# GAIA-vision/GAIA-seg

Hardware: AMD Instinct MI355X
Metric: supernet train images/sec at 1024x512 (higher is better)
Workload: dtype fp32

## Files before the change

### gaia_seg_amd/core/bricks.py

```python
import math
import warnings

import os

import torch
import torch.nn as nn
from torch.nn.modules.batchnorm import _BatchNorm

from ..hip import ops
from ..hip import runtime as _runtime
from ..hip.runtime import round_up, tape_function
from .dynamic import DynamicMixin
from .registry import Registry, build_from_cfg

CONV_LAYERS = Registry("conv layer")
NORM_LAYERS = Registry("norm layer")
ACTIVATION_LAYERS = Registry("activation layer")
ACTIVATION_LAYERS.register_module("ReLU", module=nn.ReLU)


def _nhwc_tape_call(run, x):
    if x.dim() != 4:
        raise ValueError("expected a [N, H, W, C] tensor (got %dD input)" % x.dim())
    return tape_function(lambda tape, acts: [run(tape, acts[0])], [x.permute(0, 3, 1, 2)],
# ... 383 lines not shown


_NO_FUSED_CALLS = os.environ.get("GS_NO_FUSED_CALLS") is not None


def fused_call_ok(conv, norm):
    return (conv._parameters["bias"] is None and conv.width_state % 4 == 0 and not conv.depthwise
            and not conv.__dict__.get("_deploying", False)
            and not norm.__dict__.get("_deploying", False) and not _NO_FUSED_CALLS
            and not (norm.training and norm.sync is not None and norm._process_group() is not None))


def conv_bn_act(tape, conv, norm, x, relu=False, residual=None, out=None, tag=None, defer=False,
                owns_input_grad=False, defer_residual=False):
    c = conv.width_state
    cd = conv.__dict__
    weight = conv._parameters["weight"]
    fused = (conv._parameters["bias"] is None and c % 4 == 0 and not cd.get("_deploying", False)
             and not cd["depthwise"]
             and not norm.__dict__.get("_deploying", False) and not _NO_FUSED_CALLS)
    if fused:
        bnp = norm.bn_params(c)
        if bnp.process_group is None:
            if cd.get("_layout_ptr") != weight.data_ptr():
                conv._check_layout()
                weight = conv._parameters["weight"]
                cd["_layout_ptr"] = weight.data_ptr()
            return ops.conv_bn(tape, x, weight, c, bnp, conv.stride, conv.padding,
                               conv.dilation, relu=relu, residual=residual, out=out, tag=tag,
                               defer=defer, owns_input_grad=owns_input_grad,
                               defer_residual=defer_residual)
    y = conv.forward_act(tape, x, tag=tag)
    return norm.forward_act(tape, y, relu=relu, residual=residual, out=out)


class DynamicConvModule(nn.Module, DynamicMixin):
    search_space = {"width"}

    def __init__(self, in_channels, out_channels, kernel_size, stride=1, padding=0, dilation=1,
                 groups=1, bias="auto", conv_cfg=None, norm_cfg=None, act_cfg=dict(type="ReLU"),
                 inplace=True, order=("conv", "norm", "act")):
        super().__init__()
        if tuple(order) != ("conv", "norm", "act"):
            raise NotImplementedError("only the conv-norm-act order is used by the heads")
        self.with_norm = norm_cfg is not None
        self.with_activation = act_cfg is not None
        if self.with_activation and act_cfg.get("type") != "ReLU":
            raise NotImplementedError("only ReLU activations are fused")
        if bias == "auto":
            bias = not self.with_norm
        self.with_bias = bias
        if self.with_norm and self.with_bias:
            warnings.warn("ConvModule has norm and bias at the same time")
        self.conv = build_conv_layer(conv_cfg, in_channels, out_channels, kernel_size,
                                     stride=stride, padding=padding, dilation=dilation,
                                     groups=groups, bias=bias)
        self.in_channels, self.out_channels = in_channels, out_channels
        self.inplace = inplace
        if self.with_norm:
            self.norm_name, norm = build_norm_layer(norm_cfg, out_channels)
            self.add_module(self.norm_name, norm)
        else:
            self.norm_name = None
        if self.with_activation:
            self.activate = nn.ReLU(inplace=inplace)
        self.init_weights()
# ... 190 lines not shown
```

### gaia_seg_amd/csrc/fused_layers.hip

```cpp
#include <vector>
#include "common.h"
#include "fused_internal.h"

using namespace gs;

static inline size_t align256(size_t v) { return (v + 255) & ~(size_t)255; }

extern "C" size_t gs_conv_bn_workspace_bytes(const gs_conv_desc* d) {
  if (!d) return 0;
  const size_t a = gs_conv2d_workspace_bytes(d);
  const int64_t rows = (int64_t)d->N * d->Ho * d->Wo;
  const size_t b = gs_bn_stats_workspace_bytes(rows, d->Co);
  const size_t fused = align256(a) + bn_fused_reduce_bytes(rows, d->Co);
  const size_t tiles = align256(a) + (size_t)3 * d->Co * ((rows + 63) / 64) * sizeof(float);
  size_t m = a > b ? a : b;
  if (fused > m) m = fused;
  if (tiles > m) m = tiles;
  const size_t bnb = dgrad_bnbwd_part_bytes(d);
  if (bnb > m) m = bnb;
  return m;
}

extern "C" int gs_conv_bn_forward(const gs_conv_desc* d, const float* x, const float* w,
                                  const gs_bn_args* bn, const float* residual, int32_t ld_res,
// ... 58 lines not shown
  if (input_bn && input_bn->reserved != 0) return GS_E_BADARG;
  const int64_t rows = (int64_t)d->N * d->Ho * d->Wo;
  const int32_t C = d->Co;
  int rc = GS_OK;
  if (!sums_ready) {
    rc = gs_bn_bwd_reduce(dz, ld_dz, y, d->ldy, z, ldz, rows, C, coeffs, mask_mode,
                          write_g ? dz : nullptr, ld_dz, bsums, workspace, workspace_bytes, stream);
    if (rc != GS_OK) return rc;
  }
  rc = gs_bn_bwd_apply(dz, ld_dz, y, d->ldy, z, ldz, rows, C, coeffs, bsums, (double)rows,
                       (write_g || sums_ready) ? 0 : mask_mode, bn->use_batch_stats, dy, d->ldy,
                       dgamma, dbeta, stream);
  if (rc != GS_OK) return rc;
  if (dw) {
    if (side_stream) {
      rc = gs_stream_fork(stream, side_stream);
      if (rc != GS_OK) return rc;
      rc = gs_conv2d_wgrad(d, x, dy, dw, side_workspace, side_workspace_bytes, side_stream);
    } else {
      rc = gs_conv2d_wgrad(d, x, dy, dw, workspace, workspace_bytes, stream);
    }
    if (rc != GS_OK) return rc;
  }
  if (input_bn && input_bn->fused) *input_bn->fused = 0;
  if (dx) {
    int fused = 0;
    rc = conv2d_dgrad_impl(d, dy, w, dx, accumulate_dx, workspace, workspace_bytes, stream, input_bn,
                           &fused);
    if (input_bn && input_bn->fused) *input_bn->fused = fused;
  }
  return rc;
}

namespace gs {
struct K3Prof {
  bool on = false;
  std::vector<hipEvent_t> pool;
  size_t used = 0;
  double flops = 0.0;
};
static K3Prof g_k3;
bool k3_prof_on() { return g_k3.on; }
static hipEvent_t k3_event() {
  if (g_k3.used == g_k3.pool.size()) {
    hipEvent_t e;
    if (hipEventCreate(&e) != hipSuccess) return nullptr;
    g_k3.pool.push_back(e);
  }
  return g_k3.pool[g_k3.used++];
}
struct K3Pending {
  hipEvent_t e0 = nullptr, e1 = nullptr;
  bool open = false, start_set = false, stop_set = false;
};
static thread_local K3Pending t_k3;
void k3_prof_begin(hipStream_t st) {
  (void)st;
  t_k3 = K3Pending{};
  t_k3.e0 = k3_event();
  t_k3.e1 = k3_event();
  t_k3.open = t_k3.e0 && t_k3.e1;
}
bool k3_launch_events(hipStream_t st, bool single_kernel, hipEvent_t* e0, hipEvent_t* e1) {
  if (!t_k3.open || t_k3.start_set) return false;
  static const bool markers = getenv("GS_K3_TIMER_MARKERS") != nullptr;
  t_k3.start_set = true;
// ... 42 lines not shown
```

### gaia_seg_amd/csrc/norm.hip

```cpp
#include <algorithm>
#include "common.h"
#include "fused_internal.h"

namespace gs {

struct ColMap {
  int cq;
  int rr;
  int rpi;
  bool active;
};

__device__ __forceinline__ ColMap col_map(int C4) {
  ColMap m;
  const int t = threadIdx.x;
  if (C4 <= 256) {
    m.rpi = 256 / C4;
    m.rr = t / C4;
    m.cq = t - m.rr * C4;
    m.active = m.rr < m.rpi;
  } else {
    m.rpi = 1;
    m.rr = 0;
    m.cq = blockIdx.y * 256 + t;
// ... 278 lines not shown
}

template <int MASK, bool BATCH>
__global__ __launch_bounds__(256) void bn_bwd_apply_kernel(
    const float* __restrict__ dy, int ld_dy, const float* __restrict__ x, int ldx,
    const float* __restrict__ act, int ld_act, long rows, int C, const float* __restrict__ coeffs,
    const float* __restrict__ sums, float inv_count, float* __restrict__ dx, int ld_dx,
    float* dgamma, float* dbeta) {
  const int C4 = C >> 2;
  const ColMap m = col_map(C4);
  if (!m.active) return;
  const f32x4 scale = *reinterpret_cast<const f32x4*>(coeffs + m.cq * 4);
  const f32x4 beta = *reinterpret_cast<const f32x4*>(coeffs + C + m.cq * 4);
  const f32x4 mean = *reinterpret_cast<const f32x4*>(coeffs + 2 * C + m.cq * 4);
  const f32x4 invstd = *reinterpret_cast<const f32x4*>(coeffs + 3 * C + m.cq * 4);
  const f32x4 sg = *reinterpret_cast<const f32x4*>(sums + m.cq * 4);
  const f32x4 sgx = *reinterpret_cast<const f32x4*>(sums + C + m.cq * 4);
  if (blockIdx.x == 0 && m.rr == 0) {
    if (dgamma) *reinterpret_cast<f32x4*>(dgamma + m.cq * 4) = sgx;
    if (dbeta) *reinterpret_cast<f32x4*>(dbeta + m.cq * 4) = sg;
  }
  const f32x4 c1 = sg * inv_count, c2 = sgx * inv_count;
  const long step = (long)gridDim.x * m.rpi;
  for (long r = (long)blockIdx.x * m.rpi + m.rr; r < rows; r += step) {
    const f32x4 xv = *reinterpret_cast<const f32x4*>(x + r * ldx + m.cq * 4);
    f32x4 g = *reinterpret_cast<const f32x4*>(dy + r * ld_dy + m.cq * 4);
    f32x4 av{0.f, 0.f, 0.f, 0.f};
    if (MASK == 2) av = *reinterpret_cast<const f32x4*>(act + r * ld_act + m.cq * 4);
    g = masked_grad<MASK>(g, xv, av, mean, scale, beta);
    f32x4 o;
    if (BATCH) o = scale * (g - c1 - ((xv - mean) * invstd) * c2);
    else o = scale * g;
    *reinterpret_cast<f32x4*>(dx + r * ld_dx + m.cq * 4) = o;
  }
}

__global__ __launch_bounds__(256) void colsum_partial_kernel(const float* __restrict__ x, long rows,
                                                             int C, int ldx, long rows_per_block,
                                                             float* __restrict__ part) {
  __shared__ f32x4 sh[512];
  const int C4 = C >> 2;
  const ColMap m = col_map(C4);
  f32x4 s1{0.f, 0.f, 0.f, 0.f}, s2{0.f, 0.f, 0.f, 0.f};
  if (m.active) {
    const long r0 = (long)blockIdx.x * rows_per_block;
    const long r1 = min(r0 + rows_per_block, rows);
    for (long r = r0 + m.rr; r < r1; r += m.rpi)
      s1 += *reinterpret_cast<const f32x4*>(x + r * ldx + m.cq * 4);
  }
  block_reduce_rows(s1, s2, m, C4, sh);
  if (m.active && m.rr == 0)
    reinterpret_cast<f32x4*>(part)[(long)m.cq * gridDim.x + blockIdx.x] = s1;
}


__device__ __forceinline__ void block_sum_d4(double (&a)[4], double* sh ) {
  const int lane = threadIdx.x & 63, wave = threadIdx.x >> 6;
#pragma unroll
  for (int off = 32; off > 0; off >>= 1)
#pragma unroll
    for (int e = 0; e < 4; ++e) a[e] += __shfl_xor(a[e], off, 64);
  __syncthreads();
  if (lane == 0)
#pragma unroll
    for (int e = 0; e < 4; ++e) sh[wave * 4 + e] = a[e];
  __syncthreads();
// ... 506 lines not shown
  hipLaunchKernelGGL(colsum_partial_kernel, dim3(g.gx, g.gy), dim3(256), 0, st, src, (long)rows, C,
                     ld, g.rows_per_block, part);
  launch_sum_partials(part, g.gx, C, out, nullptr, 0, st);
  return launch_status();
}

extern "C" int gs_bn_sync_local(const float* sums, double count, int32_t C, double* local,
                                void* stream) {
  if (!sums || !local) return GS_E_NULL;
  if (C <= 0 || count <= 0.0) return GS_E_BADARG;
  hipLaunchKernelGGL(bn_sync_local_kernel, dim3((C + 255) / 256), dim3(256), 0, as_stream(stream),
                     sums, count, C, local);
  return launch_status();
}

extern "C" int gs_bn_sync_merge(const double* gathered, int32_t world, int32_t C, float* merged,
                                void* stream) {
  if (!gathered || !merged) return GS_E_NULL;
  if (C <= 0 || world <= 0) return GS_E_BADARG;
  hipLaunchKernelGGL(bn_sync_merge_kernel, dim3((C + 255) / 256), dim3(256), 0, as_stream(stream),
                     gathered, world, C, merged);
  return launch_status();
}

extern "C" int gs_bn_calib_fold(const GsBnCalibLayer* layers, int32_t n_layers, float* bank,
                                int64_t bank_floats, int32_t op, float scale, void* stream) {
  if (!layers || !bank) return GS_E_NULL;
  if (n_layers <= 0 || bank_floats <= 0 || op < GS_BN_CALIB_SAVE || op > GS_BN_CALIB_WRITE)
    return GS_E_BADARG;
  hipLaunchKernelGGL(bn_calib_fold_kernel, dim3(n_layers), dim3(256), 0, as_stream(stream), layers,
                     bank, (long)bank_floats, (int)op, scale);
  return launch_status();
}
```

### gaia_seg_amd/hip/lib.py

```python
import ctypes
import os
import subprocess
from ctypes import (POINTER, Structure, c_char_p, c_double, c_float, c_int32, c_int64, c_size_t,
                    c_void_p)

_HERE = os.path.dirname(os.path.abspath(__file__))
PKG_ROOT = os.path.dirname(_HERE)
REPO_ROOT = os.path.dirname(PKG_ROOT)
LIB_PATH = os.path.join(PKG_ROOT, "lib", "libgaiaseg_hip.so")
CSRC_DIR = os.path.join(PKG_ROOT, "csrc")
ABI_VERSION = 21


class HipLibraryError(RuntimeError):
    pass


class ConvDesc(Structure):
    _fields_ = [("N", c_int32), ("H", c_int32), ("W", c_int32), ("Ci", c_int32), ("Co", c_int32),
                ("Ci_max", c_int32), ("Co_ld", c_int32), ("KH", c_int32), ("KW", c_int32),
                ("stride", c_int32), ("pad", c_int32), ("dil", c_int32), ("Ho", c_int32),
                ("Wo", c_int32), ("x_sn", c_int64), ("x_sh", c_int64), ("x_sw", c_int64),
                ("x_sc", c_int64), ("ldy", c_int32), ("ld_add", c_int32),
                ("role", c_int32), ("reserved", c_int32), ("in_affine", c_void_p)]
# ... 299 lines not shown
    "gs_sgd_set_hyper": (_i32, [_P, _f32, _f32, _f32, _f32, _P]),
    "gs_sgd_set_group_hyper": (_i32, [_P, _f32, _f32, _i32, SgdGroups, _P]),
    "gs_sgd_step_groups": (_i32, [_P, _P, _P, _P, _i32, _P, _i32, _P]),
    "gs_adamw_set_group_hyper": (_i32, [_P, _f64, _f64, _f64, _f64, _i32, AdamwGroups, _P]),
    "gs_adamw_step_groups": (_i32, [_P, _P, _P, _P, _P, _i32, _P, _i32, _P, _i32, _P]),
    "gs_grad_accumulate": (_i32, [_P, _P, _i64, _P]),
    "gs_debug_force_plan": (_i32, [_i32, _i32, _i32]),
    "gs_debug_query_plan": (_i32, [_i32, _i32, _i32, _i32, POINTER(_i32), POINTER(_i32), POINTER(_i32),
                                   POINTER(_i32)]),
    "gs_debug_last_conv_launch": (_i32, [POINTER(DebugLaunch)]),
    "gs_debug_conv_launch_counts": (_i32, [POINTER(_i64), _i32]),
    "gs_debug_k3_flops": (_i32, [POINTER(_f64), _i32]),
    "gs_debug_set_x3_fwd": (_i32, [_i32]),
    "gs_debug_set_splitk_inkernel": (_i32, [_i32]),
    "gs_debug_splitk_combined": (_i64, [_i32]),
    "gs_debug_set_col_finalize": (_i32, [_i32]),
    "gs_debug_col_finalized": (_i64, [_i32]),
    "gs_debug_num_cu": (_i32, []),
    "gs_debug_set_stream_mode": (_i32, [_i32]),
    "gs_debug_conv_launch_flops": (_i32, [POINTER(_f64), _i32]),
    "gs_debug_query_conv_launch": (_i32, [_CD, _i32, POINTER(DebugLaunch)]),
    "gs_debug_f16_launches": (_i32, [POINTER(_i64), POINTER(_f64), _i32]),
    "gs_set_forward_precision": (_i32, [_i32]),
    "gs_get_forward_precision": (_i32, []),
    "gs_set_train_precision": (_i32, [_i32]),
    "gs_get_train_precision": (_i32, []),
    "gs_debug_f16_launches_by_op": (_i32, [POINTER(_i64), POINTER(_f64), _i32]),
    "gs_stream_fork": (_i32, [_P, _P]),
    "gs_conv_bn_workspace_bytes": (_sz, [_CD]),
    "gs_conv_bn_forward": (_i32, [_CD, _P, _P, _BN, _P, _i32, _P, _P, _P, _i32, _P, _sz, _P]),
    "gs_conv_bn_backward": (_i32, [_CD, _P, _P, _P, _P, _i32, _P, _BN, _P, _i32, _i32, _i32, _P, _P,
                                   _P, _P, _P, _P, _i32, _P, _sz, _P, _sz, _P, _P, POINTER(BnBwdFuse),
                                   _i32]),
    "gs_k3_timer_enable": (_i32, [_i32]),
    "gs_k3_timer_read": (_i32, [POINTER(_i64), POINTER(_f64), POINTER(_f64)]),
}

_lib = None


def build(verbose=False, jobs=None):
    jobs = jobs or min(8, os.cpu_count() or 1)
    cmd = ["make", "-C", CSRC_DIR, "-j%d" % jobs]
    res = subprocess.run(cmd, stdout=subprocess.PIPE, stderr=subprocess.STDOUT, text=True)
    if verbose or res.returncode != 0:
        print(res.stdout)
    if res.returncode != 0:
        raise HipLibraryError("building libgaiaseg_hip.so failed (exit %d)" % res.returncode)
    global _lib
    _lib = None
    return LIB_PATH


def load():
    global _lib, LIB_PATH
    if _lib is not None:
        return _lib
    if os.environ.get("GS_HIP_LIB"):
        LIB_PATH = os.environ["GS_HIP_LIB"]
    if not os.path.exists(LIB_PATH):
        raise HipLibraryError(
            "%s not found: the HIP extension is required (no CPU fallback). Build it with "
            "`python -c 'import __graft_entry__ as g; g.build()'` or `make -C gaia_seg_amd/csrc`."
            % LIB_PATH)
    try:
        lib = ctypes.CDLL(LIB_PATH)
# ... 48 lines not shown
```

### gaia_seg_amd/hip/ops.py

```python
import ctypes

import torch

import os

from . import lib as _lib
from .runtime import WORKSPACE, Act, _Workspace, current_stream_ptr, round_up

_ws = WORKSPACE

class _DeviceStreams:
    __slots__ = ("side", "side_dirty", "branch", "origin", "branch_dirty")

    def __init__(self):
        self.side = None
        self.side_dirty = False
        self.branch = {}
        self.origin = {}
        self.branch_dirty = set()


_streams = {}


# ... 1231 lines not shown
        if residual is not None and residual.requires_grad:
            _pass_residual_grad(L, residual, dz, rows, C, s)

    tape.record(backward)
    return out


def maxpool(tape, x, k=3, s=2, p=1):
    L = _L()
    dev = x.t.device
    ho, wo = (x.H + 2 * p - k) // s + 1, (x.W + 2 * p - k) // s + 1
    out = Act.empty(x.N, ho, wo, x.C, dev)
    idx = torch.empty((x.N, ho, wo, x.C), dtype=torch.uint8, device=dev)
    _lib.check(L.gs_maxpool_forward(x.ptr, x.N, x.H, x.W, x.C, x.ld, k, s, p, ho, wo, out.ptr,
                                    out.ld, idx.data_ptr(), current_stream_ptr()),
               "gs_maxpool_forward")
    if POOL_TRACE is not None:
        POOL_TRACE.append(idx)

    def backward():
        dy = out.g
        if dy is None or not x.requires_grad:
            return
        acc = _input_grad(x)
        _lib.check(L.gs_maxpool_backward(dy.data_ptr(), dy.stride(2), idx.data_ptr(), x.N, x.H, x.W,
                                         x.C, k, s, p, ho, wo, x.g.data_ptr(), x.g.stride(2),
                                         acc, current_stream_ptr()),
                   "gs_maxpool_backward")

    tape.record(backward)
    return out


def avgpool_ceil(tape, x, s):
    L = _L()
    x = materialize(tape, x)
    dev = x.t.device
    ho, wo = (x.H + s - 1) // s, (x.W + s - 1) // s
    out = Act.empty(x.N, ho, wo, x.C, dev)
    _lib.check(L.gs_avgpool_ceil_forward(x.ptr, x.N, x.H, x.W, x.C, x.ld, s, out.ptr, out.ld,
                                         current_stream_ptr()), "gs_avgpool_ceil_forward")

    def backward():
        dy = out.g
        if dy is None or not x.requires_grad:
            return
        acc = _input_grad(x)
        _lib.check(L.gs_avgpool_ceil_backward(dy.data_ptr(), dy.stride(2), x.N, x.H, x.W, x.C, s,
                                              x.g.data_ptr(), x.g.stride(2), acc,
                                              current_stream_ptr()), "gs_avgpool_ceil_backward")

    tape.record(backward)
    return out


def copy_into(tape, x, dst):
    L = _L()
    _lib.check(L.gs_copy2d(x.ptr, x.ld, dst.ptr, dst.ld, x.rows, x.C, 1.0, 0, current_stream_ptr()),
               "gs_copy2d")

    def backward():
        dg = dst.g
        if dg is None or not x.requires_grad:
            return
        acc = _input_grad(x)
        _lib.check(L.gs_copy2d(dg.data_ptr(), dg.stride(2), x.g.data_ptr(), x.g.stride(2), x.rows,
# ... 143 lines not shown
```

### gaia_seg_amd/models/backbones/dynamic_resnet.py

```python
from collections.abc import Sequence

import torch.nn as nn
from torch.nn.modules.batchnorm import _BatchNorm

from ...core.bricks import (DynamicBatchNorm2d, DynamicBottleneck, DynamicConv2d,
                            build_conv_layer, build_norm_layer, constant_init, conv_bn_act, kaiming_init)
from ...core.dynamic import DynamicMixin, freeze, unzip_meta
from ...hip import ops
from ...hip.runtime import tape_function
from ..builder import BACKBONES
from ..utils import DynamicResLayer


@BACKBONES.register_module()
class DynamicResNet(nn.Module, DynamicMixin):
    search_space = {"stem", "body"}

    def init_state(self, stem=None, body=None, **kwargs):
        if stem is not None:
            self.stem_state = stem
        if body is not None:
            self.body_state = body
        for k, v in kwargs.items():
            setattr(self, "%s_state" % k, v)

    def __init__(self, in_channels, stem_width, body_width, body_depth, num_stages=4,
                 strides=(1, 2, 2, 2), dilations=(1, 1, 1, 1), out_indices=(0, 1, 2, 3),
                 style="pytorch", deep_stem=False, avg_down=False, frozen_stages=-1,
                 frozen_layers=None, conv_cfg=None, norm_cfg=dict(type="DynSyncBN"),
                 act_cfg=dict(type="ReLU"), norm_eval=False, dcn=None,
                 stage_with_dcn=(False, False, False, False), plugins=None, with_cp=False,
                 zero_init_residual=True, contract_dilation=False):
        super().__init__()
        if not 1 <= num_stages <= 4:
            raise AssertionError("num_stages must be in 1..4")
        if not (len(strides) == len(dilations) == num_stages) or max(out_indices) >= num_stages:
            raise AssertionError("strides / dilations / out_indices do not match num_stages")
        if dcn is not None or plugins is not None:
            raise NotImplementedError("dcn / plugins are not used by the in-tree seg configs")
# ... 81 lines not shown
            raise TypeError("pretrained must be a str or None")
        last_norms = {id(m.norm3) for m in self.modules()
                      if isinstance(m, DynamicBottleneck)} if self.zero_init_residual else set()
        for m in self.modules():
            if isinstance(m, DynamicConv2d):
                kaiming_init(m)
            elif isinstance(m, (_BatchNorm, nn.GroupNorm)):
                constant_init(m, 0 if id(m) in last_norms else 1)

    def train(self, mode=True):
        super().train(mode)
        self._freeze_stages()
        if mode and self.norm_eval:
            for m in self.modules():
                if isinstance(m, _BatchNorm):
                    m.eval()
        return self

    def _stem_convs(self):
        return [self.stem[0], self.stem[3], self.stem[6]] if self.deep_stem else [self.conv1]

    def manipulate_stem(self, arch_meta):
        self.stem_state = arch_meta
        metas = unzip_meta(arch_meta) if self.deep_stem else [arch_meta]
        for conv, meta in zip(self._stem_convs(), metas):
            conv.manipulate_arch(meta)

    def manipulate_body(self, arch_meta):
        self.body_state = arch_meta
        for name, meta in zip(self.res_layers, unzip_meta(arch_meta)):
            getattr(self, name).manipulate_arch(meta)

    def forward_act(self, tape, x):
        if self.deep_stem:
            mods = list(self.stem)
            for i in range(0, len(mods), 3):
                x = conv_bn_act(tape, mods[i], mods[i + 1], x, relu=True)
        else:
            x = conv_bn_act(tape, self.conv1, self.norm1, x, relu=True)
        mp = self.maxpool
        x = ops.maxpool(tape, x, mp.kernel_size, mp.stride, mp.padding)
        outs = []
        for i, layer_name in enumerate(self.res_layers):
            x = getattr(self, layer_name).forward_act(tape, x)
            if i == 0:
                ops.side_checkpoint(tape)
            if i in self.out_indices:
                outs.append(x)
        return outs

    def late_gradient_parameters(self):
        mods = [self.stem] if self.deep_stem else [self.conv1, self.norm1]
        mods.append(getattr(self, self.res_layers[0]))
        return [p for m in mods for p in m.parameters()]

    def forward(self, x):
        needs = any(p.requires_grad for p in self.parameters())
        return tuple(tape_function(lambda tape, acts: self.forward_act(tape, acts[0]), [x], needs))

    def active_modules(self):
        mods = [self.stem] if self.deep_stem else [self.conv1, self.norm1]
        for layer_name in self.res_layers:
            mods.extend(getattr(self, layer_name).active_blocks())
        return mods
```

### include/gaiaseg_hip.h

```cpp
#ifndef GAIASEG_HIP_H
#define GAIASEG_HIP_H

#include <stddef.h>
#include <stdint.h>

#ifdef __cplusplus
extern "C" {
#endif

#define GS_OK 0
#define GS_E_BADARG (-1)
#define GS_E_ALIGN (-2)
#define GS_E_WORKSPACE (-3)
#define GS_E_NULL (-4)

int gs_abi_version(void);
const char* gs_error_string(int code);
const char* gs_target_arch(void);

typedef struct gs_conv_desc {
  int32_t N, H, W;
  int32_t Ci, Co;
  int32_t Ci_max, Co_ld;
  int32_t KH, KW;
// ... 102 lines not shown
size_t gs_bn_stats_workspace_bytes(int64_t rows, int32_t C);
int gs_bn_stats(const float* x, int64_t rows, int32_t C, int32_t ldx, float* sums,
                void* workspace, size_t workspace_bytes, void* stream);
int gs_bn_finalize(const float* sums, double count, int32_t C, const float* gamma,
                   const float* beta, float eps, float momentum, float* running_mean,
                   float* running_var, float* coeffs, void* stream);
int gs_bn_sync_local(const float* sums, double count, int32_t C, double* local, void* stream);
int gs_bn_sync_merge(const double* gathered, int32_t world, int32_t C, float* merged, void* stream);
int gs_bn_stats_finalize(const float* x, int64_t rows, int32_t C, int32_t ldx, const float* gamma,
                         const float* beta, float eps, float momentum, float* running_mean,
                         float* running_var, float* coeffs, void* workspace,
                         size_t workspace_bytes, void* stream);
int gs_bn_eval_coeffs(const float* running_mean, const float* running_var, int32_t C,
                      const float* gamma, const float* beta, float eps, float* coeffs,
                      void* stream);
int gs_bn_apply(const float* x, int64_t rows, int32_t C, int32_t ldx, const float* coeffs,
                const float* residual, int32_t ld_res, int32_t relu, float* y, int32_t ldy,
                void* stream);
int gs_bn_apply_mask(const float* x, int64_t rows, int32_t C, int32_t ldx, const float* coeffs,
                     const float* residual, int32_t ld_res, float* y, int32_t ldy, uint8_t* mask,
                     void* stream);

size_t gs_bn_bwd_workspace_bytes(int64_t rows, int32_t C);
int gs_bn_bwd_reduce(const float* dy, int32_t ld_dy, const float* x, int32_t ldx,
                     const float* act, int32_t ld_act, int64_t rows, int32_t C,
                     const float* coeffs, int32_t mask_mode, float* g_out, int32_t ld_g,
                     float* sums, void* workspace, size_t workspace_bytes, void* stream);
int gs_bn_bwd_apply(const float* dy, int32_t ld_dy, const float* x, int32_t ldx,
                    const float* act, int32_t ld_act, int64_t rows, int32_t C,
                    const float* coeffs, const float* sums, double count, int32_t mask_mode,
                    int32_t use_batch_stats, float* dx, int32_t ld_dx, float* dgamma,
                    float* dbeta, void* stream);

typedef struct GsBnCalibLayer {
  float* running_mean;
  float* running_var;
  int32_t channels;
  int32_t offset;
} GsBnCalibLayer;
#define GS_BN_CALIB_SAVE 0
#define GS_BN_CALIB_ADD 1
#define GS_BN_CALIB_WRITE 2
int gs_bn_calib_fold(const GsBnCalibLayer* layers, int32_t n_layers, float* bank,
                     int64_t bank_floats, int32_t op, float scale, void* stream);

typedef struct gs_bn_args {
  const float* gamma;
  const float* beta;
  float* running_mean;
  float* running_var;
  float eps, momentum;
  int32_t use_batch_stats;
  int32_t update_running;
  int32_t relu;
  int32_t reserved;
  uint8_t* relu_mask;
  const float* residual_coeffs;
} gs_bn_args;
size_t gs_conv_bn_workspace_bytes(const gs_conv_desc* d);
int gs_conv_bn_forward(const gs_conv_desc* d, const float* x, const float* w, const gs_bn_args* bn,
                       const float* residual, int32_t ld_res, float* y, float* coeffs, float* z,
                       int32_t ldz, void* workspace, size_t workspace_bytes, void* stream);
typedef struct gs_bn_bwd_fuse {
  const float* y;
  const float* act;
  const float* coeffs;
  float* sums;
  int32_t* fused;
  int32_t ldy, ldact;
  int32_t mode;
  int32_t reserved;
  const uint8_t* mask;
  int32_t ldmask;
  int32_t reserved2;
} gs_bn_bwd_fuse;
int gs_conv_bn_backward(const gs_conv_desc* d, const float* x, const float* w, const float* y,
                        const float* z, int32_t ldz, const float* coeffs, const gs_bn_args* bn,
                        float* dz, int32_t ld_dz, int32_t mask_mode, int32_t write_g, float* dy,
                        float* bsums, float* dgamma, float* dbeta, float* dw, float* dx,
                        int32_t accumulate_dx, void* workspace, size_t workspace_bytes,
                        void* side_workspace, size_t side_workspace_bytes, void* stream,
                        void* side_stream, const gs_bn_bwd_fuse* input_bn, int32_t sums_ready);

int gs_k3_timer_enable(int32_t on);
int gs_k3_timer_read(int64_t* launches, double* total_ms, double* total_flops);

int gs_avgpool_ceil_forward(const float* x, int32_t N, int32_t H, int32_t W, int32_t C, int32_t ldx,
                            int32_t s, float* y, int32_t ldy, void* stream);
int gs_avgpool_ceil_backward(const float* dy, int32_t ld_dy, int32_t N, int32_t H, int32_t W,
                             int32_t C, int32_t s, float* dx, int32_t ld_dx, int32_t accumulate,
                             void* stream);
int gs_maxpool_forward(const float* x, int32_t N, int32_t H, int32_t W, int32_t C, int32_t ldx,
                       int32_t k, int32_t s, int32_t p, int32_t Ho, int32_t Wo, float* y,
                       int32_t ldy, uint8_t* idx, void* stream);
int gs_maxpool_backward(const float* dy, int32_t ld_dy, const uint8_t* idx, int32_t N, int32_t H,
                        int32_t W, int32_t C, int32_t k, int32_t s, int32_t p, int32_t Ho,
                        int32_t Wo, float* dx, int32_t ld_dx, int32_t accumulate, void* stream);

size_t gs_adaptive_avgpool_workspace_bytes(int32_t N, int32_t H, int32_t W, int32_t C,
                                           const int32_t* scales, int32_t nscales);
int gs_adaptive_avgpool_forward(const float* x, int32_t N, int32_t H, int32_t W, int32_t C,
                                int32_t ldx, const int32_t* scales, int32_t nscales, float* y,
                                void* workspace, size_t workspace_bytes, void* stream);
int gs_adaptive_avgpool_backward(const float* dy, int32_t N, int32_t H, int32_t W, int32_t C,
                                 const int32_t* scales, int32_t nscales, float* dx, int32_t ld_dx,
                                 int32_t accumulate, void* stream);

int gs_bilinear_forward(const float* x, int32_t N, int32_t Hi, int32_t Wi, int32_t C, int32_t ldx,
                        int32_t Ho, int32_t Wo, int32_t align_corners, float* y, int32_t ldy,
                        int32_t accumulate, void* stream);
size_t gs_bilinear_backward_workspace_bytes(int32_t N, int32_t Hi, int32_t Wi, int32_t C,
                                            int32_t Ho, int32_t Wo);
int gs_bilinear_backward(const float* dy, int32_t ld_dy, int32_t N, int32_t Hi, int32_t Wi,
                         int32_t C, int32_t Ho, int32_t Wo, int32_t align_corners, float* dx,
                         int32_t ld_dx, int32_t accumulate, void* workspace,
// ... 252 lines not shown
```

Measured before the change: 145.8.

## Fuse stem BN-ReLU apply into maxpool forward and backward

```diff
diff --git a/gaia_seg_amd/core/bricks.py b/gaia_seg_amd/core/bricks.py
--- a/gaia_seg_amd/core/bricks.py
+++ b/gaia_seg_amd/core/bricks.py
@@ -439,6 +439,27 @@
                                defer_residual=defer_residual)
     y = conv.forward_act(tape, x, tag=tag)
     return norm.forward_act(tape, y, relu=relu, residual=residual, out=out)
+
+
+def conv_bn_relu_maxpool(tape, conv, norm, x, pool):
+    c = conv.width_state
+    cd = conv.__dict__
+    k, s, p = pool.kernel_size, pool.stride, pool.padding
+    if (ops.STEM_POOL_FUSE and tape.enabled and conv._parameters["bias"] is None and c % 4 == 0
+            and not cd.get("_deploying", False) and not cd["depthwise"]
+            and not norm.__dict__.get("_deploying", False) and not _NO_FUSED_CALLS
+            and pool.dilation == 1 and not pool.ceil_mode):
+        bnp = norm.bn_params(c)
+        if ops.stem_pool_fusable(tape, c, bnp, True, k, s, p):
+            weight = conv._parameters["weight"]
+            if cd.get("_layout_ptr") != weight.data_ptr():
+                conv._check_layout()
+                weight = conv._parameters["weight"]
+                cd["_layout_ptr"] = weight.data_ptr()
+            return ops.conv_bn_maxpool(tape, x, weight, c, bnp, conv.stride, conv.padding,
+                                       conv.dilation, k, s, p)
+    x = conv_bn_act(tape, conv, norm, x, relu=True)
+    return ops.maxpool(tape, x, k, s, p)
 
 
 class DynamicConvModule(nn.Module, DynamicMixin):
diff --git a/gaia_seg_amd/csrc/fused_layers.hip b/gaia_seg_amd/csrc/fused_layers.hip
--- a/gaia_seg_amd/csrc/fused_layers.hip
+++ b/gaia_seg_amd/csrc/fused_layers.hip
@@ -114,6 +114,59 @@
   return rc;
 }
 
+extern "C" int gs_conv_bn_pool_forward(const gs_conv_desc* d, const float* x, const float* w,
+                                       const gs_bn_args* bn, float* y, float* coeffs, int32_t pool_k,
+                                       int32_t pool_s, int32_t pool_p, int32_t Hp, int32_t Wp,
+                                       float* pooled, int32_t ld_pooled, uint8_t* idx,
+                                       void* workspace, size_t workspace_bytes, void* stream) {
+  if (!d || !bn || !coeffs) return GS_E_NULL;
+  if (!bn->relu || !bn->use_batch_stats || bn->residual_coeffs || bn->relu_mask) return GS_E_BADARG;
+  int rc = gs_conv_bn_forward(d, x, w, bn, nullptr, 0, y, coeffs, nullptr, 0, workspace,
+                              workspace_bytes, stream);
+  if (rc != GS_OK) return rc;
+  return gs_bn_relu_pool_forward(y, d->N, d->Ho, d->Wo, d->Co, d->ldy, coeffs, pool_k, pool_s,
+                                 pool_p, Hp, Wp, pooled, ld_pooled, idx, stream);
+}
+
+extern "C" int gs_conv_bn_pool_backward(const gs_conv_desc* d, const float* x, const float* w,
+                                        const float* y, const float* coeffs, const gs_bn_args* bn,
+                                        const float* dpooled, int32_t ld_dpooled, const uint8_t* idx,
+                                        int32_t pool_k, int32_t pool_s, int32_t pool_p, int32_t Hp,
+                                        int32_t Wp, float* dy, float* bsums, float* dgamma,
+                                        float* dbeta, float* dw, float* dx, int32_t accumulate_dx,
+                                        void* workspace, size_t workspace_bytes,
+                                        void* side_workspace, size_t side_workspace_bytes,
+                                        void* stream, void* side_stream) {
+  if (!d || !bn || !coeffs || !dpooled || !idx || !dy || !bsums) return GS_E_NULL;
+  if (!bn->relu || !bn->use_batch_stats) return GS_E_BADARG;
+  const int64_t rows = (int64_t)d->N * d->Ho * d->Wo;
+  const int32_t C = d->Co;
+  int rc = gs_bn_relu_pool_bwd_reduce(dpooled, ld_dpooled, idx, y, d->ldy, d->N, d->Ho, d->Wo, C,
+                                      coeffs, pool_k, pool_s, pool_p, Hp, Wp, bsums, workspace,
+                                      workspace_bytes, stream);
+  if (rc != GS_OK) return rc;
+  rc = gs_bn_relu_pool_bwd_apply(dpooled, ld_dpooled, idx, y, d->ldy, d->N, d->Ho, d->Wo, C, coeffs,
+                                 bsums, (double)rows, pool_k, pool_s, pool_p, Hp, Wp, dy, d->ldy,
+                                 dgamma, dbeta, stream);
+  if (rc != GS_OK) return rc;
+  if (dw) {
+    if (side_stream) {
+      rc = gs_stream_fork(stream, side_stream);
+      if (rc != GS_OK) return rc;
+      rc = gs_conv2d_wgrad(d, x, dy, dw, side_workspace, side_workspace_bytes, side_stream);
+    } else {
+      rc = gs_conv2d_wgrad(d, x, dy, dw, workspace, workspace_bytes, stream);
+    }
+    if (rc != GS_OK) return rc;
+  }
+  if (dx) {
+    int fused = 0;
+    rc = conv2d_dgrad_impl(d, dy, w, dx, accumulate_dx, workspace, workspace_bytes, stream, nullptr,
+                           &fused);
+  }
+  return rc;
+}
+
 namespace gs {
 struct K3Prof {
   bool on = false;
diff --git a/gaia_seg_amd/csrc/norm.hip b/gaia_seg_amd/csrc/norm.hip
--- a/gaia_seg_amd/csrc/norm.hip
+++ b/gaia_seg_amd/csrc/norm.hip
@@ -334,6 +334,199 @@
     if (BATCH) o = scale * (g - c1 - ((xv - mean) * invstd) * c2);
     else o = scale * g;
     *reinterpret_cast<f32x4*>(dx + r * ld_dx + m.cq * 4) = o;
+  }
+}
+
+struct PoolGeom {
+  int N, H, W, Ho, Wo, k, s, p;
+};
+
+constexpr int kPoolTile = 8;
+constexpr int kPoolRowsInFlight = 2;
+
+template <bool FIX>
+__global__ __launch_bounds__(256) void bn_relu_pool_fwd_kernel(
+    const float* __restrict__ y, int ldy, int C, const float* __restrict__ coeffs, PoolGeom q,
+    int tiles_h, int tiles_w, float* __restrict__ out, int ld_out, uint8_t* __restrict__ idx) {
+  const int C4 = C >> 2;
+  const ColMap m = col_map(C4);
+  if (!m.active) return;
+  const int k = FIX ? 3 : q.k, s = FIX ? 2 : q.s, p = FIX ? 1 : q.p;
+  int b = blockIdx.x;
+  const int tw = b % tiles_w;
+  b /= tiles_w;
+  const int th = b % tiles_h;
+  const int n = b / tiles_h;
+  const f32x4 scale = *reinterpret_cast<const f32x4*>(coeffs + m.cq * 4);
+  const f32x4 beta = *reinterpret_cast<const f32x4*>(coeffs + C + m.cq * 4);
+  const f32x4 mean = *reinterpret_cast<const f32x4*>(coeffs + 2 * C + m.cq * 4);
+  const float ninf = -__builtin_huge_valf();
+  for (int px = m.rr; px < kPoolTile * kPoolTile; px += m.rpi) {
+    const int ho = th * kPoolTile + px / kPoolTile, wo = tw * kPoolTile + px % kPoolTile;
+    if (ho >= q.Ho || wo >= q.Wo) continue;
+    f32x4 best{ninf, ninf, ninf, ninf};
+    int bi[4] = {-1, -1, -1, -1};
+    if (FIX) {
+      f32x4 v[9];
+      bool inb[9];
+#pragma unroll
+      for (int t = 0; t < 9; ++t) {
+        const int h = ho * 2 - 1 + t / 3, w = wo * 2 - 1 + t % 3;
+        inb[t] = (unsigned)h < (unsigned)q.H && (unsigned)w < (unsigned)q.W;
+        const int hc = min(max(h, 0), q.H - 1), wc = min(max(w, 0), q.W - 1);
+        v[t] = *reinterpret_cast<const f32x4*>(y + ((long)(n * q.H + hc) * q.W + wc) * ldy + m.cq * 4);
+      }
+#pragma unroll
+      for (int t = 0; t < 9; ++t) {
+        f32x4 a = (v[t] - mean) * scale + beta;
+        a[0] = fmaxf(a[0], 0.f); a[1] = fmaxf(a[1], 0.f);
+        a[2] = fmaxf(a[2], 0.f); a[3] = fmaxf(a[3], 0.f);
+#pragma unroll
+        for (int e = 0; e < 4; ++e)
+          if (inb[t] && (bi[e] < 0 || a[e] > best[e] || a[e] != a[e])) { best[e] = a[e]; bi[e] = t; }
+      }
+    } else {
+      for (int kh = 0; kh < k; ++kh) {
+        const int h = ho * s - p + kh;
+        if ((unsigned)h >= (unsigned)q.H) continue;
+        for (int kw = 0; kw < k; ++kw) {
+          const int w = wo * s - p + kw;
+          if ((unsigned)w >= (unsigned)q.W) continue;
+          f32x4 a = *reinterpret_cast<const f32x4*>(y + ((long)(n * q.H + h) * q.W + w) * ldy + m.cq * 4);
+          a = (a - mean) * scale + beta;
+          a[0] = fmaxf(a[0], 0.f); a[1] = fmaxf(a[1], 0.f);
+          a[2] = fmaxf(a[2], 0.f); a[3] = fmaxf(a[3], 0.f);
+          const int tap = kh * k + kw;
+#pragma unroll
+          for (int e = 0; e < 4; ++e)
+            if (bi[e] < 0 || a[e] > best[e] || a[e] != a[e]) { best[e] = a[e]; bi[e] = tap; }
+        }
+      }
+    }
+    const long o = (long)(n * q.Ho + ho) * q.Wo + wo;
+    *reinterpret_cast<f32x4*>(out + o * ld_out + m.cq * 4) = best;
+    uchar4 bb;
+    bb.x = (uint8_t)bi[0]; bb.y = (uint8_t)bi[1]; bb.z = (uint8_t)bi[2]; bb.w = (uint8_t)bi[3];
+    *reinterpret_cast<uchar4*>(idx + (o * C4 + m.cq) * 4) = bb;
+  }
+}
+
+struct PoolTaps {
+  f32x4 d[4];
+  uchar4 b[4];
+  int code[4];
+};
+template <bool FIX>
+__device__ __forceinline__ void pool_taps_load(PoolTaps& t, const float* __restrict__ dpool, int ld_dp,
+                                               const uint8_t* __restrict__ idx, int C4,
+                                               const PoolGeom& q, int n, int h, int w, int cq) {
+  const int k = FIX ? 3 : q.k, s = FIX ? 2 : q.s, p = FIX ? 1 : q.p;
+  int ho_lo = h + p - k + 1 + s - 1;
+  ho_lo = ho_lo <= 0 ? 0 : ho_lo / s;
+  int wo_lo = w + p - k + 1 + s - 1;
+  wo_lo = wo_lo <= 0 ? 0 : wo_lo / s;
+  const int ho_hi = min((h + p) / s, q.Ho - 1), wo_hi = min((w + p) / s, q.Wo - 1);
+#pragma unroll
+  for (int j = 0; j < 4; ++j) {
+    const int ho = ho_lo + (j >> 1), wo = wo_lo + (j & 1);
+    const bool ok = ho <= ho_hi && wo <= wo_hi;
+    t.code[j] = ok ? (h - (ho * s - p)) * k + (w - (wo * s - p)) : 255;
+    const long o = (long)(n * q.Ho + min(ho, q.Ho - 1)) * q.Wo + min(wo, q.Wo - 1);
+    t.b[j] = *reinterpret_cast<const uchar4*>(idx + (o * C4 + cq) * 4);
+    t.d[j] = *reinterpret_cast<const f32x4*>(dpool + o * ld_dp + cq * 4);
+  }
+}
+__device__ __forceinline__ f32x4 pool_taps_sum(const PoolTaps& t) {
+  f32x4 g{0.f, 0.f, 0.f, 0.f};
+#pragma unroll
+  for (int j = 0; j < 4; ++j) {
+    g[0] += t.b[j].x == t.code[j] ? t.d[j][0] : 0.f;
+    g[1] += t.b[j].y == t.code[j] ? t.d[j][1] : 0.f;
+    g[2] += t.b[j].z == t.code[j] ? t.d[j][2] : 0.f;
+    g[3] += t.b[j].w == t.code[j] ? t.d[j][3] : 0.f;
+  }
+  return g;
+}
+
+template <bool FIX>
+__global__ __launch_bounds__(256) void bn_pool_bwd_partial_kernel(
+    const float* __restrict__ dpool, int ld_dp, const uint8_t* __restrict__ idx,
+    const float* __restrict__ x, int ldx, int rows, int C, const float* __restrict__ coeffs,
+    PoolGeom q, int rows_per_block, float* __restrict__ part) {
+  __shared__ f32x4 sh[512];
+  const int C4 = C >> 2;
+  const ColMap m = col_map(C4);
+  f32x4 s1{0.f, 0.f, 0.f, 0.f}, s2{0.f, 0.f, 0.f, 0.f};
+  if (m.active) {
+    const f32x4 scale = *reinterpret_cast<const f32x4*>(coeffs + m.cq * 4);
+    const f32x4 beta = *reinterpret_cast<const f32x4*>(coeffs + C + m.cq * 4);
+    const f32x4 mean = *reinterpret_cast<const f32x4*>(coeffs + 2 * C + m.cq * 4);
+    const f32x4 invstd = *reinterpret_cast<const f32x4*>(coeffs + 3 * C + m.cq * 4);
+    const int r0 = blockIdx.x * rows_per_block;
+    const int r1 = min(r0 + rows_per_block, rows);
+    for (int r = r0 + m.rr; r < r1; r += kPoolRowsInFlight * m.rpi) {
+      f32x4 xv[kPoolRowsInFlight];
+      PoolTaps taps[kPoolRowsInFlight];
+      bool live[kPoolRowsInFlight];
+#pragma unroll
+      for (int u = 0; u < kPoolRowsInFlight; ++u) {
+        const int ru = r + u * m.rpi;
+        live[u] = ru < r1;
+        const int ra = live[u] ? ru : r;
+        const int w = ra % q.W, t = ra / q.W;
+        const int h = t % q.H, n = t / q.H;
+        xv[u] = *reinterpret_cast<const f32x4*>(x + (long)ra * ldx + m.cq * 4);
+        pool_taps_load<FIX>(taps[u], dpool, ld_dp, idx, C4, q, n, h, w, m.cq);
+      }
+      __builtin_amdgcn_sched_barrier(0);
+#pragma unroll
+      for (int u = 0; u < kPoolRowsInFlight; ++u) {
+        f32x4 g = masked_grad<1>(pool_taps_sum(taps[u]), xv[u], xv[u], mean, scale, beta);
+        if (!live[u]) g = f32x4{0.f, 0.f, 0.f, 0.f};
+        s1 += g;
+        s2 += g * ((xv[u] - mean) * invstd);
+      }
+    }
+  }
+  block_reduce_rows(s1, s2, m, C4, sh);
+  if (m.active && m.rr == 0) {
+    f32x4* part4 = reinterpret_cast<f32x4*>(part);
+    part4[(long)m.cq * gridDim.x + blockIdx.x] = s1;
+    part4[((long)C4 + m.cq) * gridDim.x + blockIdx.x] = s2;
+  }
+}
+
+template <bool FIX>
+__global__ __launch_bounds__(256) void bn_pool_bwd_apply_kernel(
+    const float* __restrict__ dpool, int ld_dp, const uint8_t* __restrict__ idx,
+    const float* __restrict__ x, int ldx, int rows, int C, const float* __restrict__ coeffs,
+    const float* __restrict__ sums, float inv_count, PoolGeom q, float* __restrict__ dx, int ld_dx,
+    float* dgamma, float* dbeta) {
+  const int C4 = C >> 2;
+  const ColMap m = col_map(C4);
+  if (!m.active) return;
+  const f32x4 scale = *reinterpret_cast<const f32x4*>(coeffs + m.cq * 4);
+  const f32x4 beta = *reinterpret_cast<const f32x4*>(coeffs + C + m.cq * 4);
+  const f32x4 mean = *reinterpret_cast<const f32x4*>(coeffs + 2 * C + m.cq * 4);
+  const f32x4 invstd = *reinterpret_cast<const f32x4*>(coeffs + 3 * C + m.cq * 4);
+  const f32x4 sg = *reinterpret_cast<const f32x4*>(sums + m.cq * 4);
+  const f32x4 sgx = *reinterpret_cast<const f32x4*>(sums + C + m.cq * 4);
+  if (blockIdx.x == 0 && m.rr == 0) {
+    if (dgamma) *reinterpret_cast<f32x4*>(dgamma + m.cq * 4) = sgx;
+    if (dbeta) *reinterpret_cast<f32x4*>(dbeta + m.cq * 4) = sg;
+  }
+  const f32x4 c1 = sg * inv_count, c2 = sgx * inv_count;
+  const int step = gridDim.x * m.rpi;
+  for (int r = blockIdx.x * m.rpi + m.rr; r < rows; r += step) {
+    const int w = r % q.W, t = r / q.W;
+    const int h = t % q.H, n = t / q.H;
+    const f32x4 xv = *reinterpret_cast<const f32x4*>(x + (long)r * ldx + m.cq * 4);
+    PoolTaps taps;
+    pool_taps_load<FIX>(taps, dpool, ld_dp, idx, C4, q, n, h, w, m.cq);
+    __builtin_amdgcn_sched_barrier(0);
+    const f32x4 g = masked_grad<1>(pool_taps_sum(taps), xv, xv, mean, scale, beta);
+    const f32x4 o = scale * (g - c1 - ((xv - mean) * invstd) * c2);
+    *reinterpret_cast<f32x4*>(dx + (long)r * ld_dx + m.cq * 4) = o;
   }
 }
 
@@ -906,3 +1099,96 @@
                      bank, (long)bank_floats, (int)op, scale);
   return launch_status();
 }
+
+static int check_pool(const PoolGeom& q, int C) {
+  if (q.N <= 0 || q.H <= 0 || q.W <= 0 || C <= 0 || q.k <= 0 || q.s <= 0 || q.p < 0)
+    return GS_E_BADARG;
+  if (q.k > 15 || q.k > 2 * q.s || 2 * q.p > q.k || q.H + 2 * q.p < q.k || q.W + 2 * q.p < q.k) return GS_E_BADARG;
+  if (q.Ho != (q.H + 2 * q.p - q.k) / q.s + 1 || q.Wo != (q.W + 2 * q.p - q.k) / q.s + 1)
+    return GS_E_BADARG;
+  if ((int64_t)q.N * q.H * q.W > ((int64_t)1 << 30)) return GS_E_BADARG;
+  if ((C >> 2) > 256) return GS_E_BADARG;
+  return GS_OK;
+}
+static inline bool pool_k3s2p1(const PoolGeom& q) { return q.k == 3 && q.s == 2 && q.p == 1; }
+
+extern "C" int gs_bn_relu_pool_forward(const float* y, int32_t N, int32_t H, int32_t W, int32_t C,
+                                       int32_t ldy, const float* coeffs, int32_t k, int32_t s,
+                                       int32_t p, int32_t Ho, int32_t Wo, float* out, int32_t ld_out,
+                                       uint8_t* idx, void* stream) {
+  const PoolGeom q{N, H, W, Ho, Wo, k, s, p};
+  int rc = check_pool(q, C);
+  if (rc) return rc;
+  if ((rc = check_rows(y, (long)N * H * W, C, ldy))) return rc;
+  if ((rc = check_rows(out, (long)N * Ho * Wo, C, ld_out))) return rc;
+  if (!coeffs || !idx) return GS_E_NULL;
+  if (!aligned16(coeffs) || (reinterpret_cast<uintptr_t>(idx) & 3u)) return GS_E_ALIGN;
+  const int tiles_h = (int)ceil_div(Ho, kPoolTile), tiles_w = (int)ceil_div(Wo, kPoolTile);
+  const dim3 grid((unsigned)((long)N * tiles_h * tiles_w));
+  hipStream_t st = as_stream(stream);
+  if (pool_k3s2p1(q))
+    hipLaunchKernelGGL(bn_relu_pool_fwd_kernel<true>, grid, dim3(256), 0, st, y, ldy, C, coeffs, q,
+                       tiles_h, tiles_w, out, ld_out, idx);
+  else
+    hipLaunchKernelGGL(bn_relu_pool_fwd_kernel<false>, grid, dim3(256), 0, st, y, ldy, C, coeffs, q,
+                       tiles_h, tiles_w, out, ld_out, idx);
+  return launch_status();
+}
+
+extern "C" int gs_bn_relu_pool_bwd_reduce(const float* dpool, int32_t ld_dpool, const uint8_t* idx,
+                                          const float* y, int32_t ldy, int32_t N, int32_t H,
+                                          int32_t W, int32_t C, const float* coeffs, int32_t k,
+                                          int32_t s, int32_t p, int32_t Ho, int32_t Wo, float* sums,
+                                          void* workspace, size_t workspace_bytes, void* stream) {
+  const PoolGeom q{N, H, W, Ho, Wo, k, s, p};
+  int rc = check_pool(q, C);
+  if (rc) return rc;
+  const long rows = (long)N * H * W;
+  if ((rc = check_rows(y, rows, C, ldy))) return rc;
+  if ((rc = check_rows(dpool, (long)N * Ho * Wo, C, ld_dpool))) return rc;
+  if (!idx || !coeffs || !sums || !workspace) return GS_E_NULL;
+  if (!aligned16(coeffs) || !aligned16(workspace) || (reinterpret_cast<uintptr_t>(idx) & 3u))
+    return GS_E_ALIGN;
+  const RedGeom g = red_geom(rows, C);
+  if ((size_t)g.gx * 2 * C * sizeof(float) > workspace_bytes) return GS_E_WORKSPACE;
+  hipStream_t st = as_stream(stream);
+  float* part = static_cast<float*>(workspace);
+  if (pool_k3s2p1(q))
+    hipLaunchKernelGGL(bn_pool_bwd_partial_kernel<true>, dim3(g.gx, g.gy), dim3(256), 0, st, dpool,
+                       ld_dpool, idx, y, ldy, (int)rows, C, coeffs, q, (int)g.rows_per_block, part);
+  else
+    hipLaunchKernelGGL(bn_pool_bwd_partial_kernel<false>, dim3(g.gx, g.gy), dim3(256), 0, st, dpool,
+                       ld_dpool, idx, y, ldy, (int)rows, C, coeffs, q, (int)g.rows_per_block, part);
+  launch_sum_partials(part, g.gx, 2 * C, sums, nullptr, 0, st);
+  return launch_status();
+}
+
+extern "C" int gs_bn_relu_pool_bwd_apply(const float* dpool, int32_t ld_dpool, const uint8_t* idx,
+                                         const float* y, int32_t ldy, int32_t N, int32_t H,
+                                         int32_t W, int32_t C, const float* coeffs,
+                                         const float* sums, double count, int32_t k, int32_t s,
+                                         int32_t p, int32_t Ho, int32_t Wo, float* dy, int32_t ld_dy,
+                                         float* dgamma, float* dbeta, void* stream) {
+  const PoolGeom q{N, H, W, Ho, Wo, k, s, p};
+  int rc = check_pool(q, C);
+  if (rc) return rc;
+  const long rows = (long)N * H * W;
+  if ((rc = check_rows(y, rows, C, ldy))) return rc;
+  if ((rc = check_rows(dy, rows, C, ld_dy))) return rc;
+  if ((rc = check_rows(dpool, (long)N * Ho * Wo, C, ld_dpool))) return rc;
+  if (count <= 0.0) return GS_E_BADARG;
+  if (!idx || !coeffs || !sums) return GS_E_NULL;
+  if (!aligned16(coeffs) || !aligned16(sums) || (dgamma && !aligned16(dgamma)) ||
+      (dbeta && !aligned16(dbeta)) || (reinterpret_cast<uintptr_t>(idx) & 3u))
+    return GS_E_ALIGN;
+  const dim3 grid(apply_grid(rows, C));
+  hipStream_t st = as_stream(stream);
+  const float inv = (float)(1.0 / count);
+  if (pool_k3s2p1(q))
+    hipLaunchKernelGGL(bn_pool_bwd_apply_kernel<true>, grid, dim3(256), 0, st, dpool, ld_dpool, idx, y,
+                       ldy, (int)rows, C, coeffs, sums, inv, q, dy, ld_dy, dgamma, dbeta);
+  else
+    hipLaunchKernelGGL(bn_pool_bwd_apply_kernel<false>, grid, dim3(256), 0, st, dpool, ld_dpool, idx, y,
+                       ldy, (int)rows, C, coeffs, sums, inv, q, dy, ld_dy, dgamma, dbeta);
+  return launch_status();
+}
diff --git a/gaia_seg_amd/hip/lib.py b/gaia_seg_amd/hip/lib.py
--- a/gaia_seg_amd/hip/lib.py
+++ b/gaia_seg_amd/hip/lib.py
@@ -355,6 +355,17 @@
     "gs_conv_bn_backward": (_i32, [_CD, _P, _P, _P, _P, _i32, _P, _BN, _P, _i32, _i32, _i32, _P, _P,
                                    _P, _P, _P, _P, _i32, _P, _sz, _P, _sz, _P, _P, POINTER(BnBwdFuse),
                                    _i32]),
+    "gs_bn_relu_pool_forward": (_i32, [_P, _i32, _i32, _i32, _i32, _i32, _P, _i32, _i32, _i32, _i32,
+                                       _i32, _P, _i32, _P, _P]),
+    "gs_bn_relu_pool_bwd_reduce": (_i32, [_P, _i32, _P, _P, _i32, _i32, _i32, _i32, _i32, _P, _i32,
+                                          _i32, _i32, _i32, _i32, _P, _P, _sz, _P]),
+    "gs_bn_relu_pool_bwd_apply": (_i32, [_P, _i32, _P, _P, _i32, _i32, _i32, _i32, _i32, _P, _P, _f64,
+                                         _i32, _i32, _i32, _i32, _i32, _P, _i32, _P, _P, _P]),
+    "gs_conv_bn_pool_forward": (_i32, [_CD, _P, _P, _BN, _P, _P, _i32, _i32, _i32, _i32, _i32, _P,
+                                       _i32, _P, _P, _sz, _P]),
+    "gs_conv_bn_pool_backward": (_i32, [_CD, _P, _P, _P, _P, _BN, _P, _i32, _P, _i32, _i32, _i32,
+                                        _i32, _i32, _P, _P, _P, _P, _P, _P, _i32, _P, _sz, _P, _sz,
+                                        _P, _P]),
     "gs_k3_timer_enable": (_i32, [_i32]),
     "gs_k3_timer_read": (_i32, [POINTER(_i64), POINTER(_f64), POINTER(_f64)]),
 }
diff --git a/gaia_seg_amd/hip/ops.py b/gaia_seg_amd/hip/ops.py
--- a/gaia_seg_amd/hip/ops.py
+++ b/gaia_seg_amd/hip/ops.py
@@ -1287,6 +1287,88 @@
     return out
 
 
+STEM_POOL_FUSE = os.environ.get("GS_STEM_POOL_FUSE", "1") != "0"
+
+
+def stem_pool_fusable(tape, co, bn, relu, k, s, p):
+    return bool(STEM_POOL_FUSE and relu and tape.enabled and RELU_TRACE is None and co % 4 == 0
+                and co <= 1024 and (k, s, p) == (3, 2, 1) and bn.process_group is None
+                and (bn.training or bn.running_mean is None)
+                and _L().gs_get_train_precision() == _lib.PRECISION_FP32)
+
+
+def conv_bn_maxpool(tape, x, weight, co, bn, stride=1, pad=0, dil=1, k=3, s=2, p=1):
+    _check_precision(tape)
+    L = _L()
+    if not stem_pool_fusable(tape, co, bn, True, k, s, p):
+        raise ValueError("conv_bn_maxpool: not a fusable conv + BatchNorm + ReLU + MaxPool2d")
+    dev = x.t.device
+    x = materialize(tape, x)
+    pl = _conv_bn_plan(L, x, weight, co, bn, stride, pad, dil, True, None, True)
+    if pl.rows <= 1:
+        raise ValueError("Expected more than 1 value per channel when training, got input size %s"
+                         % ((pl.n, co, pl.ho, pl.wo),))
+    d, args, need, C, rows = pl.d, pl.args, pl.need, pl.C, pl.rows
+    hp, wp = (pl.ho + 2 * p - k) // s + 1, (pl.wo + 2 * p - k) // s + 1
+    y = Act.empty(pl.n, pl.ho, pl.wo, co, dev)
+    out = Act.empty(pl.n, hp, wp, co, dev)
+    idx = torch.empty((pl.n, hp, wp, co), dtype=torch.uint8, device=dev)
+    d.in_affine = None
+    _bn_pointers(args, bn)
+    args.residual_coeffs = None
+    args.relu_mask = None
+    coeffs = torch.empty(6 * C, dtype=torch.float32, device=dev)
+    ws = _ws.get(need, dev)
+    _lib.check(L.gs_conv_bn_pool_forward(ctypes.byref(d), x.ptr, weight.data_ptr(), ctypes.byref(args),
+                                         y.ptr, coeffs.data_ptr(), k, s, p, hp, wp, out.ptr, out.ld,
+                                         idx.data_ptr(), ws.data_ptr(), ws.numel(),
+                                         current_stream_ptr()), "gs_conv_bn_pool_forward")
+    if bn.training and bn.num_batches_tracked is not None:
+        bn.num_batches_tracked()
+    if POOL_TRACE is not None:
+        POOL_TRACE.append(idx)
+
+    def backward():
+        dp = out.g
+        if dp is None:
+            return
+        st = current_stream_ptr()
+        wgrad_bn = bn.weight is not None and bn.weight.requires_grad
+        bgrad_bn = bn.bias is not None and bn.bias.requires_grad
+        ggamma = ensure_grad(bn.weight) if wgrad_bn else None
+        gbeta = ensure_grad(bn.bias) if bgrad_bn else None
+        gw = ensure_grad(weight) if weight.requires_grad else None
+        dy = torch.empty_like(y.t)
+        acc = 0
+        dx_ptr = None
+        if x.requires_grad:
+            acc = _input_grad(x)
+            dx_ptr = x.g.data_ptr()
+        ws_b = _ws.get(need, dev)
+        queued = SIDE_WGRAD and gw is not None
+        d.in_affine = None
+        _bn_pointers(args, bn)
+        _lib.check(L.gs_conv_bn_pool_backward(
+            ctypes.byref(d), x.ptr, weight.data_ptr(), y.ptr, coeffs.data_ptr(), ctypes.byref(args),
+            dp.data_ptr(), dp.stride(2), idx.data_ptr(), k, s, p, hp, wp, dy.data_ptr(),
+            coeffs.data_ptr() + 16 * C, ggamma.data_ptr() if wgrad_bn else None,
+            gbeta.data_ptr() if bgrad_bn else None,
+            gw.data_ptr() if (gw is not None and not queued) else None,
+            dx_ptr, acc, ws_b.data_ptr(), ws_b.numel(), None, 0, st, None),
+            "gs_conv_bn_pool_backward")
+        if wgrad_bn:
+            _notify(bn.weight)
+        if bgrad_bn:
+            _notify(bn.bias)
+        if queued:
+            queue_wgrad(d, x, dy, weight, gw, need, dev)
+        elif gw is not None:
+            _notify(weight)
+
+    tape.record(backward)
+    return out
+
+
 def avgpool_ceil(tape, x, s):
     L = _L()
     x = materialize(tape, x)
diff --git a/gaia_seg_amd/models/backbones/dynamic_resnet.py b/gaia_seg_amd/models/backbones/dynamic_resnet.py
--- a/gaia_seg_amd/models/backbones/dynamic_resnet.py
+++ b/gaia_seg_amd/models/backbones/dynamic_resnet.py
@@ -4,7 +4,8 @@
 from torch.nn.modules.batchnorm import _BatchNorm
 
 from ...core.bricks import (DynamicBatchNorm2d, DynamicBottleneck, DynamicConv2d,
-                            build_conv_layer, build_norm_layer, constant_init, conv_bn_act, kaiming_init)
+                            build_conv_layer, build_norm_layer, constant_init, conv_bn_act,
+                            conv_bn_relu_maxpool, kaiming_init)
 from ...core.dynamic import DynamicMixin, freeze, unzip_meta
 from ...hip import ops
 from ...hip.runtime import tape_function
@@ -152,14 +153,14 @@
             getattr(self, name).manipulate_arch(meta)
 
     def forward_act(self, tape, x):
+        mp = self.maxpool
         if self.deep_stem:
             mods = list(self.stem)
-            for i in range(0, len(mods), 3):
+            for i in range(0, len(mods) - 3, 3):
                 x = conv_bn_act(tape, mods[i], mods[i + 1], x, relu=True)
+            x = conv_bn_relu_maxpool(tape, mods[-3], mods[-2], x, mp)
         else:
-            x = conv_bn_act(tape, self.conv1, self.norm1, x, relu=True)
-        mp = self.maxpool
-        x = ops.maxpool(tape, x, mp.kernel_size, mp.stride, mp.padding)
+            x = conv_bn_relu_maxpool(tape, self.conv1, self.norm1, x, mp)
         outs = []
         for i, layer_name in enumerate(self.res_layers):
             x = getattr(self, layer_name).forward_act(tape, x)
diff --git a/include/gaiaseg_hip.h b/include/gaiaseg_hip.h
--- a/include/gaiaseg_hip.h
+++ b/include/gaiaseg_hip.h
@@ -158,6 +158,20 @@
                     int32_t use_batch_stats, float* dx, int32_t ld_dx, float* dgamma,
                     float* dbeta, void* stream);
 
+int gs_bn_relu_pool_forward(const float* y, int32_t N, int32_t H, int32_t W, int32_t C, int32_t ldy,
+                            const float* coeffs, int32_t k, int32_t s, int32_t p, int32_t Ho,
+                            int32_t Wo, float* out, int32_t ld_out, uint8_t* idx, void* stream);
+int gs_bn_relu_pool_bwd_reduce(const float* dpool, int32_t ld_dpool, const uint8_t* idx,
+                               const float* y, int32_t ldy, int32_t N, int32_t H, int32_t W,
+                               int32_t C, const float* coeffs, int32_t k, int32_t s, int32_t p,
+                               int32_t Ho, int32_t Wo, float* sums, void* workspace,
+                               size_t workspace_bytes, void* stream);
+int gs_bn_relu_pool_bwd_apply(const float* dpool, int32_t ld_dpool, const uint8_t* idx,
+                              const float* y, int32_t ldy, int32_t N, int32_t H, int32_t W, int32_t C,
+                              const float* coeffs, const float* sums, double count, int32_t k,
+                              int32_t s, int32_t p, int32_t Ho, int32_t Wo, float* dy, int32_t ld_dy,
+                              float* dgamma, float* dbeta, void* stream);
+
 typedef struct GsBnCalibLayer {
   float* running_mean;
   float* running_var;
@@ -207,6 +221,20 @@
                         int32_t accumulate_dx, void* workspace, size_t workspace_bytes,
                         void* side_workspace, size_t side_workspace_bytes, void* stream,
                         void* side_stream, const gs_bn_bwd_fuse* input_bn, int32_t sums_ready);
+
+int gs_conv_bn_pool_forward(const gs_conv_desc* d, const float* x, const float* w,
+                            const gs_bn_args* bn, float* y, float* coeffs, int32_t pool_k,
+                            int32_t pool_s, int32_t pool_p, int32_t Hp, int32_t Wp, float* pooled,
+                            int32_t ld_pooled, uint8_t* idx, void* workspace, size_t workspace_bytes,
+                            void* stream);
+int gs_conv_bn_pool_backward(const gs_conv_desc* d, const float* x, const float* w, const float* y,
+                             const float* coeffs, const gs_bn_args* bn, const float* dpooled,
+                             int32_t ld_dpooled, const uint8_t* idx, int32_t pool_k, int32_t pool_s,
+                             int32_t pool_p, int32_t Hp, int32_t Wp, float* dy, float* bsums,
+                             float* dgamma, float* dbeta, float* dw, float* dx,
+                             int32_t accumulate_dx, void* workspace, size_t workspace_bytes,
+                             void* side_workspace, size_t side_workspace_bytes, void* stream,
+                             void* side_stream);
 
 int gs_k3_timer_enable(int32_t on);
 int gs_k3_timer_read(int64_t* launches, double* total_ms, double* total_flops);
```

Result: no change. 146.1, median of 6 (+0.2%).
